# david-cortes/recometrics

Hardware: AMD Instinct MI355X
Metric: users/sec evaluated (all metrics, K=10) (higher is better)
Workload: dtype f32

## Files before the change

recometrics_amd/csrc/rm_launch.hpp:

```cpp
#pragma once
#include "rm_device.hpp"
#include "rm_list.hpp"

namespace rm {

typedef double f64x2 __attribute__((ext_vector_type(2)));
constexpr int GROUP_USERS64 = 16;

struct SweepArgs {
    int n, K;
    int ngt;
    int ext_topk;
    int spec;
    int n_slots, n_groups, n_ublocks;
    int ublock0;
    int n_splits, tiles_total;
    int tail_ublocks, tail_splits, part_splits;
    int part_extra;
    int jmax;
    int list_in_lds;
    int check_nan;
    int buffered_lists;
    int pend_cap, pend_off;
    int sync_off;
    const float4 *Ap, *Bp;
    const int *slot_user, *slot_chunk;
    const int *train_p, *train_i;
    const unsigned *train_bits; int train_words;
    const int *gj; const long long *grow;
    const float *pos_score;
    const int *pos_item;
    unsigned *hist;
    unsigned *thr_shared;
    u32x2 *glists;
    int lane_cap; int *lane_cnt;
    ListEntry *pl;
    PartialStat<float> *pst;
    float *dump;
    int stream_slot0;
    long long stream_ld;
    float *stream_scores;
    const int *noise_row; int noise_row0; const float *noise_E; long long noise_ld;
};

struct Sweep64Args {
    int n, K;
    int ngt;
    int ext_topk;
    int spec;
    int n_slots, n_groups, n_ublocks;
    int ublock0;
// ... 45 lines not shown
```

recometrics_amd/csrc/rm_lib.hip:

```cpp
#include <hip/hip_runtime.h>

#include <algorithm>
#include <array>
#include <cmath>
#include <cstdio>
#include <cstring>
#include <cstdlib>
#include <type_traits>
#include <atomic>
#include <chrono>
#include <condition_variable>
#include <csignal>
#include <functional>
#include <limits>
#include <map>
#include <memory>
#include <mutex>
#include <string>
#include <thread>
#include <vector>

#include "../../include/recometrics_hip.h"
#include "rm_device.hpp"
#include "rm_prep.hpp"
#include "rm_launch.hpp"
#include "rm_finalize.hpp"
#include "rm_noise.hpp"
#include "rm_scores.hpp"

namespace {

using namespace rm;

thread_local std::string g_err;
struct RmError { int code; std::string msg; };

#define HIP_CHECK(expr)                                                                                   \
    do {                                                                                                  \
        hipError_t e_ = (expr);                                                                           \
        if (e_ != hipSuccess)                                                                             \
            throw RmError{e_ == hipErrorOutOfMemory ? RM_ERR_NOMEM : RM_ERR_HIP,                          \
                          std::string(#expr) + ": " + hipGetErrorString(e_)};                             \
    } while (0)

struct Switches {
    bool no_train_bits, no_spec, no_side, ext_topk, no_test_mask, hbm_lists, nsub2, no_pending, no_pos_beside, no_seed, rank_generic,
         no_fused_auc, no_defer_auc, noise_sequential, one_context, noise_per_batch, host_trace, no_pos_flat;
    long long free_mb, stream_budget_mb, noise_budget_mb, lane_cap_min, lane_min_k, lane_cap_set, sample_seed;
    double batch_users;
    std::string splits;
    static bool on(const char *name) { return getenv(name) != nullptr; }
    static long long num(const char *name) { const char *e = getenv(name); return e ? atoll(e) : -1; }
    void load()
    {
        no_train_bits = on("RM_DEBUG_NO_TRAIN_BITS"); no_spec = on("RM_DEBUG_NO_SPEC"); no_side = on("RM_DEBUG_NO_SIDE");
        ext_topk = on("RM_DEBUG_EXT_TOPK"); no_test_mask = on("RM_DEBUG_NO_TEST_MASK");
        hbm_lists = on("RM_DEBUG_HBM_LISTS"); nsub2 = on("RM_DEBUG_NSUB2"); no_pending = on("RM_DEBUG_NO_PENDING");
        no_pos_beside = on("RM_DEBUG_NO_POS_BESIDE"); no_seed = on("RM_DEBUG_NO_SEED");
        rank_generic = on("RM_DEBUG_RANK_GENERIC"); no_fused_auc = on("RM_DEBUG_NO_FUSED_AUC");
        no_defer_auc = on("RM_DEBUG_NO_DEFER_AUC"); noise_sequential = on("RM_DEBUG_NOISE_SEQUENTIAL");
        one_context = on("RM_DEBUG_ONE_CONTEXT"); noise_per_batch = on("RM_DEBUG_NOISE_PER_BATCH"); host_trace = on("RM_HOST_TRACE");
        no_pos_flat = on("RM_DEBUG_NO_POS_FLAT");
        free_mb = num("RM_DEBUG_FREE_MB"); stream_budget_mb = num("RM_STREAM_BUDGET_MB");
        noise_budget_mb = num("RM_NOISE_BUDGET_MB");
        lane_min_k = num("RM_DEBUG_LANE_MIN_K");
        lane_cap_set = num("RM_DEBUG_LANE_CAP");
        sample_seed = num("RM_DEBUG_SAMPLE_SEED");
        lane_cap_min = num("RM_DEBUG_LANE_CAP_MIN");
        const char *b = getenv("RM_BATCH_USERS"); batch_users = b ? atof(b) : 0.0;
        const char *s = getenv("RM_DEBUG_SPLITS"); splits = s ? s : "";
    }
    Switches() { load(); }
};
Switches g_sw;

std::atomic<long long> g_ws_bytes{0};
inline long long debug_free_cap()
{
    return g_sw.free_mb >= 0 ? (g_sw.free_mb << 20) : -1;
}

struct RunTrace {
    std::mutex mu; std::vector<std::pair<const char *, double>> pts; std::chrono::steady_clock::time_point t0 = std::chrono::steady_clock::now();
    void point(const char *what) { std::lock_guard<std::mutex> lk(mu); if (pts.size() > 4096) pts.clear(); pts.emplace_back(what, std::chrono::duration<double, std::milli>(std::chrono::steady_clock::now() - t0).count()); }
};
RunTrace g_run_trace;
#define RM_TRACE_POINT(what) do { if (g_sw.host_trace) g_run_trace.point(what); } while (0)

std::atomic<unsigned long long> g_ws_stamp{1};
struct Workspace {
    struct Buf { void *ptr = nullptr; size_t bytes = 0; unsigned long long stamp = 0; };
    std::map<std::string, Buf> bufs;
    void *get(const std::string &name, size_t bytes)
    {
        bytes = std::max<size_t>(bytes, 256);
// ... 309 lines not shown
{
    return lane_lists_possible<T>(K, three_subtiles) && lane_list_bytes<T>(K, lane_blocks_bound<T>(m)) <= lane_budget_bytes(ws);
}

inline long long dense_row_words(long long n) { return (n + 191) / 192 * 6; }
inline bool dense_rows_fit(const Workspace &ws, int m, long long n)
{
    const long long words = dense_row_words(n);
    if (words > TRAIN_BITS_MAX_WORDS || g_sw.no_train_bits) return false;
    const unsigned long long bytes = (unsigned long long)m * (unsigned long long)words * 4ull;
    if (bytes <= (1ull << 30)) return true;
    if (bytes > (8ull << 30)) return false;
    return (long long)bytes <= free_plus_owned(ws, {"train_bits", "stream_scores", "sel_hi", "sel_lo"}) / 4;
}
template <class C> inline void set_train_bits(SweepArgs &sa, Ctx &cx, const C &c, int m, int n, bool fit, hipStream_t stream, bool mask_test, bool early = false, bool early_masked = false,
                                              unsigned char *ent_masked = nullptr)
{
    Workspace &ws = cx.ws;
    const long long words = dense_row_words(n);
    const size_t bytes = (size_t)m * (size_t)words * 4;
    sa.train_bits = nullptr; sa.train_words = 0;
    if (!fit) { cx.dense.invalidate(); return; }
    unsigned *bits = (unsigned *)ws.get("train_bits", bytes);
    const bool ready = (early && early_masked == mask_test) || (c.same_train_rows && cx.dense.fits(ws, m, words, mask_test));
    if (!ready)
        launch_train_bits(stream, m, n, (int)words, c.train_p, c.train_i, (mask_test || ent_masked) ? c.test_p : nullptr, c.test_i, bits,
                          (const Plan *)ws.get("plan", sizeof(Plan)), c.only_users, ent_masked, mask_test);
    cx.dense.set(ws, words, m, mask_test, ready ? cx.dense.partial : c.only_users != nullptr, c.items_tag, c.train_p);
    sa.train_bits = bits; sa.train_words = (int)words;
}
template <class C> inline void set_train_bits(Sweep64Args &, Ctx &, const C &, int, int, bool, hipStream_t, bool, bool = false, bool = false, unsigned char * = nullptr) {}
inline void set_part_extra(SweepArgs &sa, int extra) { sa.part_extra = extra; }
inline void set_part_extra(Sweep64Args &, int) {}
inline void set_spec(SweepArgs &sa)
{
    sa.spec = (sa.check_nan || sa.noise_E || sa.ext_topk || g_sw.no_spec) ? 0 : (sa.train_bits ? 1 : 2);
}
inline void set_spec(Sweep64Args &sa) { sa.spec = (sa.check_nan || sa.noise_E || sa.ext_topk || g_sw.no_spec) ? 0 : 1; }
inline void set_ext_bits(SweepArgs &sa, const unsigned *bits, int words) { sa.train_bits = bits; sa.train_words = words; }
inline void set_ext_bits(Sweep64Args &, const unsigned *, int) {}

template <class T> inline int sample_seed_items(const Workspace &ws, int K, int n, long long n_slots, bool off, bool lists = false)
{
    if (off || g_sw.sample_seed == 0) return 0;
    int S;
    if (g_sw.sample_seed > 0) {
        S = 64;
        for (int c : {256, 1024, 2048, 4096}) if (g_sw.sample_seed >= c) S = c;
    } else {
        S = K <= 128 ? 1024 : (K <= 384 ? 2048 : 4096);
        if (lists) { if (K < 12) return 0; S = 256; }
        if ((long long)S * 6 > n || K * 2 > S) return 0;
        if (sizeof(T) == 8 && K < 16) return 0;
    }
    if (S > n || K > S) return 0;
    if ((long long)sizeof(T) * n_slots * S > free_plus_owned(ws, {"sample_scores"}) / 8) return 0;
    return S;
}
template <class T, class Args>
inline void seed_from_sample(const Args &sa, Workspace &ws, int S, int NG, int n_slots, int n_ublocks, hipStream_t stream, const void *items64 = nullptr, void *lists = nullptr)
{
    typedef Prec<T> P;
    typedef typename std::remove_pointer<decltype(Args{}.thr_shared)>::type ThrT;
    T *sample = (T *)ws.get("sample_scores", sizeof(T) * (size_t)n_slots * (size_t)S);
    Args sd = sa;
    sd.n = S; sd.tiles_total = S / TILE_ITEMS; sd.K = 1; sd.n_splits = 1; sd.tail_ublocks = 0; sd.tail_splits = 1; sd.part_splits = 1;
// ... 126 lines not shown
        double best = 1e300;
        for (int sct = 1; sct <= max_splits; sct++) {
            const double t1 = last((double)n_ublocks * sct / n_cu) * block(sct);
            if (t1 < best - 1e-9) { best = t1; n_splits = sct; tail_ublocks = 0; tail_splits = 0; }
            const long long full = (long long)n_ublocks * sct / n_cu;
            const int main_ub = (int)(full * n_cu / sct), tail_ub = n_ublocks - main_ub;
            if (full == 0 || tail_ub == 0) continue;
            for (int ts = sct + 1; ts <= max_tail; ts++) {
                const double t2 = (double)main_ub * sct / n_cu * block(sct) + last((double)tail_ub * ts / n_cu) * block(ts);
                if (t2 < best * 0.99) { best = t2; n_splits = sct; tail_ublocks = tail_ub; tail_splits = ts; }
            }
        }
    }
    if (!sw.splits.empty()) {
        int v[3] = {1, 0, 0};
        sscanf(sw.splits.c_str(), "%d,%d,%d", &v[0], &v[1], &v[2]);
        n_splits = std::max(1, std::min(v[0], std::max(1, MAX_PARTS / nsub)));
        tail_ublocks = std::max(0, std::min(v[1], n_ublocks)); tail_splits = std::max(1, std::min(v[2], std::max(1, MAX_PARTS / nsub)));
        if (tail_ublocks == 0) tail_splits = 0;
    }
    g.n_splits = n_splits; g.tail_ublocks = tail_ublocks; g.tail_splits = tail_splits;
    g.part_splits = std::max(n_splits, tail_splits);
    g.mask_test = std::is_same<T, float>::value && want_auc && !ext_topk && !check_nan && hp.n_slots > 0 &&
                  dense_ok && hp.n_slots == hp.n_active && hp.n_only_ndcg == 0 &&
                  nsub * g.part_splits + 1 <= MAX_PARTS && !sw.no_test_mask;
    g.use_ext_bits = c.ext_bits != nullptr && c.ext_words == dense_row_words(n) && (!c.ext_masked || g.mask_test);
    if (g.use_ext_bits) g.mask_test = c.ext_masked;
    g.n_part = nsub * g.part_splits + (g.mask_test ? 1 : 0);
    g.part_extra = g.mask_test ? 1 : 0;
    g.list_in_lds = !ext_topk && !want_lane && lds_need_n(true, nsub) + SYNC_BYTES <= LDS_LIMIT && !sw.hbm_lists;
    g.want_pending = !ext_topk && !want_lane && P::has_pending && !sw.no_pending;
    g.per_key = (size_t)g.n_waves * WAVE * P::pend_key_bytes;
    g.pend_cap = g.want_pending ? P::pend_cap_max : 0;
    g.lds_total = std::min<size_t>(LDS_LIMIT, lds_need_n(g.list_in_lds, nsub) + SYNC_BYTES + g.pend_cap * g.per_key);
    g.sync_off = g.lds_total - SYNC_BYTES;
    g.u_split = 0; g.j_shallow = -1; g.lds_l = 0;
    if (!g.list_in_lds && !want_lane && K <= 32 && want_auc && !sw.hbm_lists) {
        for (int j = g.jmax - 1; j >= 0 && g.j_shallow < 0; j--)
            if (sweep_lds<T>(NG, K, want_auc, true, nsub, j) + SYNC_BYTES <= LDS_LIMIT) g.j_shallow = j;
        if (g.j_shallow >= 0) g.u_split = hp.class_offset[g.j_shallow + 1] / (GROUPS_PER_BLOCK * P::GU);
    }
    if (g.u_split > 0)
        g.lds_l = std::min<size_t>(LDS_LIMIT, sweep_lds<T>(NG, K, want_auc, true, nsub, g.j_shallow) + SYNC_BYTES + g.pend_cap * g.per_key);
    return g;
}

inline Geometry scores_geometry(const Plan &hp, int n, bool want_auc)
{
    Geometry g{};
    g.jmax = want_auc ? hp.jmax : 0;
    g.n_ublocks = (hp.n_groups + GROUPS_PER_BLOCK - 1) / GROUPS_PER_BLOCK;
    g.nsub = 2; g.tile_items = TILE_ITEMS; g.n_waves = 8;
    g.tiles_total = (n + TILE_ITEMS - 1) / TILE_ITEMS;
    g.n_splits = 1; g.part_splits = 1; g.n_part = 1;
    g.u_split = 0; g.j_shallow = -1;
    return g;
}

template <class T>
struct Pipeline {
    typedef Prec<T> P;
    typedef typename std::remove_pointer<decltype(typename P::Args{}.thr_shared)>::type ThrT;
    static constexpr int GU = P::GU;
    const Call<T> &c; hipStream_t stream; Ctx &cx; Workspace &ws;
    const int m, n, k, K;
    const bool use_side = !g_sw.no_side;
    Beside side, pos;
// ... 241 lines not shown
        if (want_auc) positives();

        if (n_stream > 0) stream_scores = (T *)ws.get("stream_scores", sizeof(T) * (size_t)n_stream * (size_t)stream_ld);
        if (!ext_topk) pl = (Entry<T> *)ws.get("pl", sizeof(Entry<T>) * (size_t)n_slots * g.n_part * K);
        pst = (PartialStat<T> *)ws.get("pst", sizeof(PartialStat<T>) * (size_t)n_slots * g.n_part);
        const unsigned n_blocks = (unsigned)((g.n_ublocks - g.tail_ublocks) * g.n_splits + g.tail_ublocks * g.tail_splits);
        lane_lists = want_lane && !ext_topk;
        int lane_cap = lane_lists ? P::lane_cap(K) : 0;
        if (lane_lists && g_sw.lane_cap_set > 0) lane_cap = (int)std::min<long long>(std::max<long long>(P::lane_cap(K), (g_sw.lane_cap_set + 15) / 16 * 16), (COLLECT_MAX_ENTRIES - K) / 16 * 16);
        if (lane_lists && g_sw.lane_cap_min >= 0)
            lane_cap = std::min(lane_cap, (K + lane_sel_slack(K) + 16 + 1 + 15) / 16 * 16);
        if (lane_lists) {
            glists = (typename P::ListT *)ws.get("glists", (size_t)n_blocks * g.n_waves * WAVE * (size_t)lane_cap * (sizeof(T) + 4));
            lane_cnt = (int *)ws.get("lane_cnt", sizeof(int) * (size_t)n_blocks * g.n_waves * WAVE);
        } else if (!g.list_in_lds && !ext_topk) {
            glists = (typename P::ListT *)ws.get("glists", sizeof(typename P::ListT) * (size_t)n_blocks * g.n_waves * GU * (2 * K + 32));
        }

        thr_shared = (ThrT *)ws.get("thr_shared", sizeof(ThrT) * (size_t)n_slots);
        if (want_auc && !ext_topk && !g_sw.no_seed)
            hipLaunchKernelGGL((k_seed_thresholds<T, ThrT>), dim3(cdiv(n_slots, 256)), dim3(256), 0, stream, n_slots, stream_slot0, K, GU, slot_user, slot_chunk,
                               user_nslots, flags, c.test_p, grow, pos_score, spos_score, thr_shared);
        else HIP_CHECK(hipMemsetAsync(thr_shared, 0, sizeof(ThrT) * (size_t)n_slots, stream));
        sa.thr_shared = thr_shared;
        sa.n = n; sa.K = K; sa.ngt = NG; sa.n_slots = n_slots; sa.n_groups = n_groups; sa.n_ublocks = g.n_ublocks;
        sa.n_splits = g.n_splits; sa.tail_ublocks = g.tail_ublocks; sa.tail_splits = g.tail_splits; sa.part_splits = g.part_splits; sa.tiles_total = tiles_total; sa.jmax = g.jmax; sa.check_nan = check_nan ? 1 : 0; sa.buffered_lists = (want_lane || ext_topk) ? 1 : 0; sa.ext_topk = ext_topk ? 1 : 0;
        sa.Ap = (decltype(sa.Ap))Ap; sa.Bp = (decltype(sa.Bp))Bp; sa.slot_user = slot_user; sa.slot_chunk = slot_chunk;
        sa.train_p = c.train_p; sa.train_i = c.train_i; sa.gj = gj; sa.grow = grow;
        sa.pos_score = pos_score; sa.pos_item = pos_item; sa.hist = hist; sa.glists = glists; sa.lane_cap = lane_cap; sa.lane_cnt = lane_cnt; sa.pl = pl; sa.pst = pst; sa.dump = nullptr;
        P::set_pending(sa, g.pend_cap, 0);
        P::set_sync(sa, (int)g.sync_off);
        sa.stream_slot0 = stream_slot0; sa.stream_ld = stream_ld; sa.stream_scores = stream_scores;
        set_part_extra(sa, g.part_extra);
        sa.noise_row = c.noise_row; sa.noise_row0 = c.noise_row0; sa.noise_E = c.noise_E; sa.noise_ld = c.noise_ld;
        set_spec(sa);

        if (side.marked(SIDE_ROWS_AND_PACKS)) side.await(SIDE_ROWS_AND_PACKS, stream);
        const bool sample_lists = !lane_lists && !ext_topk && sizeof(T) == 4;
        const int sample_S = (lane_lists || sample_lists) ? sample_seed_items<T>(ws, K, n, n_slots, check_nan || c.noise_E != nullptr, sample_lists) : 0;
        if (sample_S > 0 && !sample_lists) seed_from_sample<T>(sa, ws, sample_S, NG, n_slots, g.n_ublocks, stream);
        else if (sample_S > 0) {
            const long long units = P::items_units(sample_S / TILE_ITEMS, NG);
            typename P::PackT *Bs = (typename P::PackT *)ws.get("sample_items", 16 * (size_t)units);
            void *Ls = ws.get("sample_lists", sizeof(typename P::ListT) * (size_t)g.n_ublocks * 8 * GU * (2 + 32));
            pack_operands(c.A, c.lda, c.B, c.ldb, sample_S, k, NG, TILE_ITEMS, slot_user, 0, Ap, 0, Bs, units, stream, true);
            seed_from_sample<T>(sa, ws, sample_S, NG, n_slots, g.n_ublocks, stream, Bs, Ls);
        }
        RM_TRACE_POINT("run: preparation enqueued");
    }

    void positives()
    {
        const int n_groups = hp.n_groups;
        const long long rows = hp.total_rows + n_groups;
        pos_score = (T *)ws.get("pos_score", sizeof(T) * (size_t)(rows + 1) * GU);
        pos_item = (int *)ws.get("pos_item", sizeof(int) * (size_t)(rows + 1) * GU);
        hist = (unsigned *)ws.get("hist", sizeof(unsigned) * (size_t)(rows + 1) * GU);
        T *pos_tmp = (T *)ws.get("pos_tmp", sizeof(T) * (size_t)std::max<long long>(c.nnz_test, 1));
        pos_order = (int *)ws.get("pos_order", sizeof(int) * (size_t)std::max<long long>(c.nnz_test, 1));
        PosArgs<T> pa{m, n, k, c.A, c.lda, c.B, c.ldb, c.train_p, c.train_i, c.test_p, c.test_i,
                      flags, user_nslots, uslot_base, slot_index, grow, pos_tmp, pos_order, pos_score, pos_item, GU};
        pa.noise_row = c.noise_row; pa.noise_row0 = c.noise_row0; pa.noise_E = c.noise_E; pa.noise_ld = c.noise_ld;
        pa.noise_flag = c.noise_flag; pa.plan = plan;
        if (sizeof(T) == 4)
            pa.pos_key = (unsigned long long *)ws.get("pos_key", 8 * ((size_t)std::max<long long>(c.nnz_test, 1) + 8));
        const bool flat = flat_early;
// ... 1384 lines not shown
```

recometrics_amd/csrc/rm_sweep.hpp:

```cpp
#pragma once
#include "rm_device.hpp"
#include "rm_list.hpp"
#include "rm_launch.hpp"

namespace rm {

typedef float f32x16 __attribute__((ext_vector_type(16)));

__device__ __forceinline__ float hw_max(float a, float b) { float d; asm("v_max_f32 %0, %1, %2" : "=v"(d) : "v"(a), "v"(b)); return d; }
__device__ __forceinline__ float hw_max3(float a, float b, float c) { float d; asm("v_max3_f32 %0, %1, %2, %3" : "=v"(d) : "v"(a), "v"(b), "v"(c)); return d; }
__device__ __forceinline__ float hw_min3(float a, float b, float c) { float d; asm("v_min3_f32 %0, %1, %2, %3" : "=v"(d) : "v"(a), "v"(b), "v"(c)); return d; }


typedef __attribute__((address_space(3))) unsigned long long *LdsListPtr;
typedef u32x2 *GblListPtr;

typedef __attribute__((address_space(3))) const float *LdsF32Ptr;
typedef __attribute__((address_space(3))) unsigned *LdsU32Ptr;

#define RM_CMP_LT(m, p, x) asm volatile("v_cmp_lt_f32 %0, %1, %2" : "=s"(m) : "v"(p), "v"(x))
#define RM_SEL(d, a, b, m) asm volatile("v_cndmask_b32 %0, %1, %2, %3" : "=v"(d) : "v"(a), "v"(b), "s"(m))
__device__ __forceinline__ float hw_absmin3(float a, float b, float c) { float d; asm("v_min3_f32 %0, |%1|, |%2|, |%3|" : "=v"(d) : "v"(a), "v"(b), "v"(c)); return d; }

template <int J>
__device__ __forceinline__ void auc_pass(const float (&v)[16], unsigned pos_addr,
                                         const int *pos_item_g, int sb, int h, float piv_root, float piv_lo, float piv_hi)
{
    constexpr unsigned HIST_DELTA = (unsigned)GROUPS_PER_BLOCK * (1u << J) * GROUP_USERS * 4u;
    unsigned at[16];
#ifndef RM_TOP_LEVELS
#define RM_TOP_LEVELS 2
#endif
    constexpr int TOP = J >= 2 ? RM_TOP_LEVELS : 0;
    unsigned long long mk0, mk1, mk2;
    if (TOP == 2) {
        constexpr unsigned Q = 128u << (J >= 2 ? J - 2 : 0);
        const unsigned a1 = pos_addr | Q, a2 = pos_addr | (2 * Q), a3 = pos_addr | (3 * Q);
        #pragma unroll
        for (int r = 0; r < 16; r++) at[r] = pos_addr;
        #pragma unroll
        for (int i = 0; i < 48 + 2; i++) {
            if (i < 48) {
                const float pv = i < 16 ? piv_lo : (i < 32 ? piv_root : piv_hi);
                if (i % 3 == 0) RM_CMP_LT(mk0, pv, v[i % 16]); else if (i % 3 == 1) RM_CMP_LT(mk1, pv, v[i % 16]); else RM_CMP_LT(mk2, pv, v[i % 16]);
            }
            if (i >= 2) {
                const int j = i - 2;
                const unsigned tgt = j < 16 ? a1 : (j < 32 ? a2 : a3);
                if (j % 3 == 0) RM_SEL(at[j % 16], at[j % 16], tgt, mk0); else if (j % 3 == 1) RM_SEL(at[j % 16], at[j % 16], tgt, mk1); else RM_SEL(at[j % 16], at[j % 16], tgt, mk2);
            }
        }
    } else if (TOP == 1) {
        const unsigned a2 = pos_addr | (128u << (J >= 1 ? J - 1 : 0));
        #pragma unroll
        for (int i = 0; i < 16 + 2; i++) {
            if (i < 16) { if (i % 3 == 0) RM_CMP_LT(mk0, piv_root, v[i]); else if (i % 3 == 1) RM_CMP_LT(mk1, piv_root, v[i]); else RM_CMP_LT(mk2, piv_root, v[i]); }
            if (i >= 2) {
                const int j = i - 2;
                if (j % 3 == 0) RM_SEL(at[j], pos_addr, a2, mk0); else if (j % 3 == 1) RM_SEL(at[j], pos_addr, a2, mk1); else RM_SEL(at[j], pos_addr, a2, mk2);
            }
        }
    } else {
        #pragma unroll
        for (int r = 0; r < 16; r++) at[r] = pos_addr;
    }
    constexpr int FIRST_ST = J - TOP > 0 ? (1 << (J - TOP - 1)) : 0;
    #pragma unroll
    for (int st = FIRST_ST; st >= 1; st >>= 1) {
        float pv[16];
        #pragma unroll
        for (int r = 0; r < 16; r++) pv[r] = *(LdsF32Ptr)(at[r] + (st - 1) * 128);
        #pragma unroll
        for (int i = 0; i < 16 + 2; i++) {
            if (i == 0) __builtin_amdgcn_s_waitcnt(0xCC7F); else if (i == 4) __builtin_amdgcn_s_waitcnt(0xC87F);
            else if (i == 8) __builtin_amdgcn_s_waitcnt(0xC47F); else if (i == 12) __builtin_amdgcn_s_waitcnt(0xC07F);
            if (i < 16) { if (i % 3 == 0) RM_CMP_LT(mk0, pv[i], v[i]); else if (i % 3 == 1) RM_CMP_LT(mk1, pv[i], v[i]); else RM_CMP_LT(mk2, pv[i], v[i]); }
            if (i >= 2) {
                const int j = i - 2;
                const unsigned cand = at[j] | (unsigned)(st * 128);
                if (j % 3 == 0) RM_SEL(at[j], at[j], cand, mk0); else if (j % 3 == 1) RM_SEL(at[j], at[j], cand, mk1); else RM_SEL(at[j], at[j], cand, mk2);
            }
        }
    }
    float nx[16];
    #pragma unroll
    for (int r = 0; r < 16; r++) nx[r] = *(LdsF32Ptr)(at[r]);
    float df[16];
    #pragma unroll
    for (int r = 0; r < 16; r++) {
        if (r == 0) __builtin_amdgcn_s_waitcnt(0xCC7F); else if (r == 4) __builtin_amdgcn_s_waitcnt(0xC87F);
        else if (r == 8) __builtin_amdgcn_s_waitcnt(0xC47F); else if (r == 12) __builtin_amdgcn_s_waitcnt(0xC07F);
        df[r] = nx[r] - v[r];
    }
    const float m0 = hw_absmin3(df[0], df[1], df[2]), m1 = hw_absmin3(df[3], df[4], df[5]), m2 = hw_absmin3(df[6], df[7], df[8]);
    const float m3 = hw_absmin3(df[9], df[10], df[11]), m4 = hw_absmin3(df[12], df[13], df[14]);
    const float dmin = hw_absmin3(hw_absmin3(m0, m1, m2), hw_absmin3(m3, m4, df[15]), df[15]);
    if (wave_any(dmin == 0.f)) {
        int sb_walk = sb;
        asm volatile("" : "+s"(sb_walk));
        auto walk = [&](int r) {
            if (df[r] == 0.f) {
                const int item = sb_walk + mfma32_row(r, h);
                unsigned t = at[r] - pos_addr;
                while (*(const int *)((const char *)pos_item_g + t) > item) {
                    t += 128;
                    if (!(t < (unsigned)(((1 << J) - 1) * 128) && *(LdsF32Ptr)(pos_addr + t) == v[r])) break;
                }
                at[r] = pos_addr + t;
            }
        };
        if (wave_any(m0 == 0.f)) { walk(0); walk(1); walk(2); }
        if (wave_any(m1 == 0.f)) { walk(3); walk(4); walk(5); }
        if (wave_any(m2 == 0.f)) { walk(6); walk(7); walk(8); }
        if (wave_any(m3 == 0.f)) { walk(9); walk(10); walk(11); }
        if (wave_any(m4 == 0.f)) { walk(12); walk(13); walk(14); }
        if (wave_any(df[15] == 0.f)) walk(15);
    }
    const unsigned one = 1u;
    #pragma unroll
    for (int r = 0; r < 16; r++)
        asm volatile("ds_add_u32 %0, %1 offset:%2" :: "v"(at[r]), "v"(one), "n"(HIST_DELTA) : "memory");
}


template <int NGT, bool AUC, bool DUMP, int LMODE, int NSUB, int SPEC = 0>
__global__ __launch_bounds__(256 * NSUB)
void k_sweep(SweepArgs a)
{
    constexpr int TILE = 32 * NSUB;
    static_assert(SPEC >= 0 && SPEC <= 2 && !(SPEC && DUMP), "unknown specialisation");
    const bool f_bits = SPEC == 1 ? true : (SPEC == 2 ? false : a.train_bits != nullptr);
    const bool f_nan = SPEC ? false : a.check_nan != 0, f_noise = SPEC ? false : a.noise_E != nullptr, f_ext = SPEC ? false : a.ext_topk != 0;
    constexpr int NWAVES = 4 * NSUB, THREADS = 64 * NWAVES;
    constexpr bool LLDS = LMODE == LM_LDS;
    constexpr bool buffered = LMODE == LM_HBM_APPEND;
    constexpr bool NGT_RT = NGT == 0;
    constexpr int NG = NGT_RT ? 16 : (NGT < 16 ? NGT : 16);
    constexpr int NC_CT = NGT_RT ? 0 : NGT / NG;
    const int NGTV = NGT_RT ? a.ngt : NGT;
    const int NC = NGT_RT ? a.ngt / NG : NC_CT;
    constexpr bool AF_RESIDENT = NC_CT == 1;
    constexpr bool AF_PREFETCH = !AF_RESIDENT && LMODE != LM_HBM_APPEND;
    extern __shared__ __attribute__((aligned(16))) char smem[];
    constexpr int BUF_F4 = NG * 2 * TILE;
    const int tid = threadIdx.x, lane = tid & 63, wave = __builtin_amdgcn_readfirstlane(tid >> 6);
    const int gi = wave & 3, sub = wave >> 2;
    const int ul = lane & 31, h = lane >> 5;
    int blk_u, split, nsplit;
    {
        const int n_ub1 = a.n_ublocks - a.tail_ublocks, b1 = n_ub1 * a.n_splits;
        if ((int)blockIdx.x < b1) { blk_u = a.ublock0 + a.n_ublocks - 1 - (int)(blockIdx.x % n_ub1); split = blockIdx.x / n_ub1; nsplit = a.n_splits; }
        else { const int j = (int)blockIdx.x - b1; blk_u = a.ublock0 + a.tail_ublocks - 1 - j % a.tail_ublocks; split = j / a.tail_ublocks; nsplit = a.tail_splits; }
    }
    const int group = blk_u * GROUPS_PER_BLOCK + gi;
    const bool group_ok = group < a.n_groups;
    const int slot = group * GROUP_USERS + ul;
    const bool slot_ok = group_ok && slot < a.n_slots;
    const int K = a.K, n = a.n;

    const int glast = min(a.n_groups, (blk_u + 1) * GROUPS_PER_BLOCK) - 1;
    const int jb = AUC ? a.gj[glast] : 0;
    const int PLb = (1 << jb) - 1;

    float4 *ldsB = (float4 *)smem;
    char *p = smem + 2 * BUF_F4 * 16;
    ListEntry *lists_lds = (ListEntry *)p;
    if (LLDS) p += GROUPS_PER_BLOCK * (K + 2) * GROUP_USERS * (int)sizeof(ListEntry);
    const int PLmax = PLb;
    const unsigned tbytes = (unsigned)(PLmax + 1) * GROUP_USERS * 4;
    p = smem + (((unsigned)(p - smem) + tbytes - 1) / tbytes) * tbytes;
    float *posL = (float *)p;  p += GROUPS_PER_BLOCK * tbytes;
    unsigned *histL = (unsigned *)p;  p += AUC ? GROUPS_PER_BLOCK * tbytes : 0;
    const int pend_room = (a.sync_off - (int)(p - smem)) / (NWAVES * WAVE * 8);
    char *pend_lds = p;

    const int user = slot_ok ? a.slot_user[slot] : -1;
    const bool primary = slot_ok && a.slot_chunk[slot] == 0;
    float thr = primary ? neg_inf_f() : nan_sentinel_f();
    float vmax = neg_inf_f(), vmin = pos_inf_f();
    bool track_min = true;
    unsigned long long nanmask = 0;
    int ntc = 0, nte = 0, nt = IDX_EMPTY, nt2 = IDX_EMPTY;

    const int tiles_per = (a.tiles_total + nsplit - 1) / nsplit;
    const int t0 = split * tiles_per, t1 = min(a.tiles_total, t0 + tiles_per);
    const int ntiles = max(0, t1 - t0);

    const unsigned *tb_row = (a.train_bits && user >= 0) ? a.train_bits + (size_t)user * a.train_words : nullptr;
    unsigned tb_idx = (a.train_bits && user >= 0) ? (unsigned)user * (unsigned)a.train_words + (unsigned)(t0 * NSUB + sub) : 0u;
    if (user >= 0 && !f_bits) {
        ntc = a.train_p[user]; nte = a.train_p[user + 1];
        const int first_item = t0 * TILE;
        int lo = ntc, hi = nte;
        while (lo < hi) { const int mid = (lo + hi) >> 1; if (a.train_i[mid] < first_item) lo = mid + 1; else hi = mid; }
        ntc = lo;
        nt = ntc < nte ? a.train_i[ntc] : IDX_EMPTY;
        nt2 = ntc + 1 < nte ? a.train_i[ntc + 1] : IDX_EMPTY;
    }

    float4 af[NG];
    const float4 *af_src = a.Ap + ((size_t)(group_ok ? group : 0) * NGTV * 2 + h) * GROUP_USERS + ul;
    #pragma unroll
// ... 30 lines not shown
    auto list_release = [&]() {
        if (!LLDS) return;
        if (h == 0) { Lwk[0] = wkey; Lwp[0] = (unsigned long long)wpos; }
        if (lane == 0) __hip_atomic_store(list_lock, 0u, __ATOMIC_RELEASE, __HIP_MEMORY_SCOPE_WORKGROUP);
    };
    const int pend_want = pend_room < a.pend_cap ? pend_room : a.pend_cap;
    const int pend_cap = (buffered || pend_want < 2) ? 0 : pend_want;
    int pcnt = 0;
    LdsListPtr Pp = (LdsListPtr)((unsigned long long *)pend_lds + wave * pend_cap * WAVE + lane);
    auto offer_key = [&](unsigned long long key) {
        if (LLDS) { keylist_offer<GROUP_USERS>(Ll, K, key, wkey, wpos); return; }
        float s; int item;
        unpack_key(key, s, item);
        if (s >= ws) list_offer<float, GROUP_USERS>(Lr, K, s, item, ws, widx, wpos);
    };
    bool merged = false;
    auto merge_pending = [&]() {
        merged = true;
        const int pc = __shfl_xor(pcnt, 32);
        const int lim = h == 0 ? (pcnt > pc ? pcnt : pc) : 0;
        list_acquire();
        for (int i = 0; wave_any(i < lim); i++) {
            if (h == 0) {
                if (i < pcnt) offer_key(Pp[i * WAVE]);
                if (i < pc) offer_key(Pp[i * WAVE + 32]);
            }
        }
        list_release();
        pcnt = 0;
        if (LLDS) ws = (wkey >> 32) ? ord_unkey((unsigned)(wkey >> 32)) : neg_inf_f();
    };

    if (AUC) {
        for (int i = tid; i < GROUPS_PER_BLOCK * (PLb + 1) * GROUP_USERS; i += THREADS) {
            const int g4 = i / ((PLb + 1) * GROUP_USERS), rem = i % ((PLb + 1) * GROUP_USERS);
            const int gg = blk_u * GROUPS_PER_BLOCK + g4;
            posL[g4 * (PLmax + 1) * GROUP_USERS + rem] = gg < a.n_groups ? a.pos_score[(a.grow[gg] + gg) * GROUP_USERS + rem] : pos_inf_f();
        }
        for (int i = tid; i < GROUPS_PER_BLOCK * (PLmax + 1) * GROUP_USERS; i += THREADS) histL[i] = 0;
    }
    const unsigned pos_addr = (unsigned)(size_t)(__attribute__((address_space(3))) const float *)(posL + gi * (PLmax + 1) * GROUP_USERS + ul);
    float piv_root = pos_inf_f(), piv_lo = pos_inf_f(), piv_hi = pos_inf_f();
    if (AUC && jb >= 2) {
        __syncthreads();
        const int r0 = (1 << (jb - 1)) - 1, d = 1 << (jb - 2);
        piv_root = *(LdsF32Ptr)(pos_addr + r0 * 128);
        piv_lo = *(LdsF32Ptr)(pos_addr + (r0 - d) * 128);
        piv_hi = *(LdsF32Ptr)(pos_addr + (r0 + d) * 128);
    }
    const int *pos_item_g = (AUC && group_ok) ? a.pos_item + (a.grow[group] + group) * GROUP_USERS + ul : nullptr;
    const bool stream_lane = slot_ok && slot >= a.stream_slot0;
    const bool wave_streams = wave_any(stream_lane);
    float *stream_row = stream_lane ? a.stream_scores + (size_t)(slot - a.stream_slot0) * (size_t)a.stream_ld : nullptr;
    const float *noise_lane = (a.noise_E && user >= 0)
        ? a.noise_E + (size_t)(a.noise_row ? a.noise_row[user] - a.noise_row0 : user) * (size_t)a.noise_ld : nullptr;

    const unsigned lds_base = (unsigned)(__UINTPTR_TYPE__)(__attribute__((address_space(3))) char *)smem;
    constexpr int STAGE_PIECES = (NG + 3) / 4;
    unsigned stage_voff[STAGE_PIECES];
    #pragma unroll
    for (int j = 0; j < STAGE_PIECES; j++) stage_voff[j] = (unsigned)(((gi + 4 * j) * 2 * TILE + h * TILE + sub * 32 + ul) * 16);
    auto stage = [&](int unit, int buf) {
        const char *src = (const char *)a.Bp + (size_t)unit * (BUF_F4 * 16);
        #pragma unroll
        for (int j = 0; j < STAGE_PIECES; j++) {
            const int g = gi + 4 * j;
            if (NG % 4 == 0 || g < NG) {
                const unsigned m0v = lds_base + (unsigned)((buf * BUF_F4 + (sub * NG + g) * 64) * 16);
                asm volatile("s_mov_b32 m0, %0\n\ts_nop 0\n\tglobal_load_lds_dwordx4 %1, %2"
                             :: "s"(m0v), "v"(stage_voff[j]), "s"(src) : "memory", "m0");
            }
        }
    };

#ifndef RM_FULL_BARRIER
    constexpr bool EARLY_ARRIVE = AF_RESIDENT && NG >= 4 && NG % 2 == 0;
#else
    constexpr bool EARLY_ARRIVE = false;
#endif
    static_assert(!EARLY_ARRIVE || NG % 2 == 0, "early arrival needs an even number of factor groups");
    LdsU32Ptr arrive_p = (LdsU32Ptr)(smem + a.sync_off) + sub;
// ... 208 lines not shown
                const unsigned long long hitm = __ballot(v[r] >= thr);
                if (hitm) {
                    const float other = (hitm >> 32) ? __shfl_xor(v[r], 32) : nan_sentinel_f();
                    if (h == 0 && primary) {
                        const int item0 = sb + mfma32_row(r, 0), item1 = sb + mfma32_row(r, 1);
                        if (LLDS) { if (v[r] >= ws) keylist_offer<GROUP_USERS>(Ll, K, pack_key(v[r], item0), wkey, wpos);
                                    if (other >= ws) keylist_offer<GROUP_USERS>(Ll, K, pack_key(other, item1), wkey, wpos);
                                    ws = (wkey >> 32) ? ord_unkey((unsigned)(wkey >> 32)) : neg_inf_f(); }
                        else      { if (v[r] >= ws) list_offer<float, GROUP_USERS>(Lr, K, v[r], item0, ws, widx, wpos);
                                    if (other >= ws) list_offer<float, GROUP_USERS>(Lr, K, other, item1, ws, widx, wpos); }
                    }
                }
            }
            list_release();
        }
        if (!buffered && cm && (!pend_cap || merged)) {
            merged = false;
            const float t2 = __shfl(ws, ul);
            if (primary) {
                thr = t2 > thr ? t2 : thr;
                const unsigned kk = ord_key(t2);
                if (h == 0 && kk > thr_pub) { atomicMax(a.thr_shared + slot, kk); }
                thr_pub = kk > thr_pub ? kk : thr_pub;
            }
        }
        if (wave_streams) {
            if (stream_lane) {
                #pragma unroll
                for (int q4 = 0; q4 < 4; q4++)
                    *(float4 *)(stream_row + sb + 8 * q4 + 4 * h) = make_float4(v[4 * q4], v[4 * q4 + 1], v[4 * q4 + 2], v[4 * q4 + 3]);
            }
        }
        if (AUC) {
            switch (jb) {
                case 1: auc_pass<1>(v, pos_addr, pos_item_g, sb, h, piv_root, piv_lo, piv_hi); break;
                case 2: auc_pass<2>(v, pos_addr, pos_item_g, sb, h, piv_root, piv_lo, piv_hi); break;
                case 3: auc_pass<3>(v, pos_addr, pos_item_g, sb, h, piv_root, piv_lo, piv_hi); break;
                case 4: auc_pass<4>(v, pos_addr, pos_item_g, sb, h, piv_root, piv_lo, piv_hi); break;
                case 5: auc_pass<5>(v, pos_addr, pos_item_g, sb, h, piv_root, piv_lo, piv_hi); break;
                case 6: auc_pass<6>(v, pos_addr, pos_item_g, sb, h, piv_root, piv_lo, piv_hi); break;
                default: break;
            }
        }
        if (buffered) {
            const bool own = wave_any(lb_off >= lb_trig_now);
            unsigned ep = __builtin_amdgcn_readfirstlane(*sel_epoch);
            if (own || (ep != sel_seen && wave_any(lb_off >= lb_half))) {
                if (own && ep == sel_seen) {
                    if (lane == 0) asm volatile("ds_add_u32 %0, %1" :: "v"((unsigned)(__UINTPTR_TYPE__)sel_epoch), "v"(1u) : "memory");
                    ep++;
                }
                lane_bounds();
                lb_trig_now = lb_trigger;
            }
            sel_seen = ep;
        }
    };

    f32x16 acc;
    const int nunits = ntiles * NC;
    constexpr unsigned SYNC_WAVES = 4;
    LdsU32Ptr arrive = (LdsU32Ptr)(smem + a.sync_off) + sub;
    if (tid < (buffered ? 8 : 4)) ((LdsU32Ptr)(smem + a.sync_off))[tid] = 0u;
    if (ntiles > 0) stage(t0 * NC, 0);
    unsigned tile_bits = (tb_row && ntiles > 0) ? a.train_bits[tb_idx] >> (4 * h) : 0u;
    __builtin_amdgcn_s_waitcnt(WAIT_VMCNT0);
    __syncthreads();
    auto load_thr = [&]() -> unsigned {
        return (primary && !DUMP) ? __hip_atomic_load(a.thr_shared + slot, __ATOMIC_RELAXED, __HIP_MEMORY_SCOPE_AGENT) : 0u;
    };
    unsigned thr_seen = load_thr();
    for (int i = 0; i < ntiles; i++) {
        unsigned thr_next = thr_seen;
// ... 16 lines not shown
                const int sub_s = __builtin_amdgcn_readfirstlane(sub);
                const unsigned mine = sub_s == 0 ? c0 : (sub_s == 1 ? c1 : c2);
                const unsigned o1 = sub_s == 0 ? c1 : c0, o2 = (NSUB == 3) ? (sub_s == 2 ? c1 : c2) : o1;
                const bool behind = mine + 2 < o1 || mine + 2 < o2, ahead = mine > o1 + 2 && mine > o2 + 2;
                if (behind) __builtin_amdgcn_s_setprio(2);
                else if (ahead) __builtin_amdgcn_s_setprio(0);
                else __builtin_amdgcn_s_setprio(1);
            }
#endif
            if (unit + 1 < nunits) stage(t0 * NC + unit + 1, (unit + 1) & 1);
            if (c == 0) thr_next = load_thr();
            unsigned bits_next = 0u;
            if (c == NC - 1 && tb_row && i + 1 < ntiles) { tb_idx += NSUB; bits_next = a.train_bits[tb_idx]; }
            do_mfma(acc, unit & 1, c, tile_bits);
#ifndef RM_FULL_BARRIER
            __builtin_amdgcn_s_waitcnt(WAIT_VMCNT0);
            if (!EARLY_ARRIVE && lane == 0) asm volatile("ds_add_u32 %0, %1" :: "v"((unsigned)(__UINTPTR_TYPE__)arrive), "v"(1u) : "memory");
#endif
            if (c == NC - 1) do_epi(acc, t0 + i, thr_seen, tile_bits);
            if (c == NC - 1) tile_bits = bits_next >> (4 * h);
#if defined(RM_FULL_BARRIER)
            __builtin_amdgcn_s_waitcnt(WAIT_VMCNT0);
            __syncthreads();
#endif
        }
        thr_seen = thr_next;
    }
    if (DUMP) return;
    if (pend_cap) merge_pending();
    if (LLDS) __syncthreads();

    {
    const SweepArgs &a = *late_kernargs<SweepArgs>();
    const int n_part = a.part_splits * NSUB + a.part_extra;
    const int part = split * NSUB + sub;
    {
        const float omax = __shfl_xor(vmax, 32), omin = __shfl_xor(vmin, 32);
        vmax = __builtin_fmaxf(vmax, omax); vmin = __builtin_fminf(vmin, omin);
        const bool hn = ((nanmask >> ul) & 1ull) | ((nanmask >> (ul + 32)) & 1ull);
        if (slot_ok && h == 0) {
            PartialStat<float> ps;
            ps.vmax = vmax; ps.vmin = vmin; ps.rocsum = 0; ps.has_nan = hn ? 1 : 0; ps.pad = 0;
            a.pst[(size_t)slot * n_part + part] = ps;
            ListEntry *dst = a.pl + ((size_t)slot * n_part + part) * K;
            if (LLDS && sub == 0) { keylist_sort_desc<GROUP_USERS>(Ll, K); for (int i = 0; i < K; i++) unpack_key(Ll[i * GROUP_USERS], dst[i].s, dst[i].idx); }
            if (LLDS && sub != 0) { dst[0].s = neg_inf_f(); dst[0].idx = IDX_EMPTY; }
            if (split == 0) for (int sp = nsplit; sp < a.part_splits; sp++) {
                ps.vmax = neg_inf_f(); ps.vmin = pos_inf_f(); ps.has_nan = 0;
                a.pst[(size_t)slot * n_part + sp * NSUB + sub] = ps;
                ListEntry *de = a.pl + ((size_t)slot * n_part + sp * NSUB + sub) * K;
                if (a.pl) { de[0].s = neg_inf_f(); de[0].idx = IDX_EMPTY; }
            }
        }
    }
    if (AUC && a.part_extra && split == 0 && sub == 0 && h == 0 && slot_ok && slot < a.stream_slot0) {
        const int pe = n_part - 1;
        ListEntry *dx = a.pl + ((size_t)slot * n_part + pe) * K;
        const unsigned hcol = (unsigned)(size_t)(__attribute__((address_space(3))) unsigned *)(histL + gi * (PLmax + 1) * GROUP_USERS + ul);
        float bmax = neg_inf_f(), bmin = pos_inf_f();
        int filled = 0;
        for (int i = PLb - 1; i >= 0; i--) {
            const float x = *(LdsF32Ptr)(pos_addr + (unsigned)i * 128u);
            if (x < pos_inf_f()) {
                if (filled == 0) bmax = x;
                bmin = x;
                asm volatile("ds_add_u32 %0, %1" :: "v"(hcol + (unsigned)i * 128u), "v"(1u) : "memory");
                if (filled < K) { dx[filled].s = x; dx[filled].idx = pos_item_g[i * GROUP_USERS]; }
                filled++;
            }
        }
        for (int i = filled; i < K; i++) { dx[i].s = neg_inf_f(); dx[i].idx = IDX_EMPTY; }
        PartialStat<float> ps;
        ps.vmax = bmax; ps.vmin = bmin; ps.rocsum = 0; ps.has_nan = 0; ps.pad = 0;
        a.pst[(size_t)slot * n_part + pe] = ps;
    }
    if (!LLDS && !buffered) {
        if (slot_ok && h == 0) {
            ListEntry *dst = a.pl + ((size_t)slot * n_part + part) * K;
            list_sort_desc<float, GROUP_USERS>(Lr, K);
            for (int i = 0; i < K; i++) ListRaw<float>::unpack(Lr[i * GROUP_USERS], dst[i].s, dst[i].idx);
        }
    } else if (!LLDS && !a.ext_topk) {
        a.lane_cnt[((size_t)blockIdx.x * NWAVES + wave) * WAVE + lane] = (slot_ok && primary) ? (int)(lb_off >> 9) : 0;
    }
    if (AUC) {
        __builtin_amdgcn_s_waitcnt(0xC07F);
        __syncthreads();
        for (int i = tid; i < GROUPS_PER_BLOCK * (PLb + 1) * GROUP_USERS; i += THREADS) {
            const int g4 = i / ((PLb + 1) * GROUP_USERS), rem = i % ((PLb + 1) * GROUP_USERS);
            const int gg = blk_u * GROUPS_PER_BLOCK + g4;
            const unsigned c = histL[g4 * (PLmax + 1) * GROUP_USERS + rem];
            if (gg < a.n_groups && c) atomicAdd(&a.hist[(a.grow[gg] + gg) * GROUP_USERS + rem], c);
        }
    }
    }
}

}
```

Measured before the change: 17.73 million.

## Store AUC positive-score table as score/next-address pairs for branchless binary search

Result: no change. 17.80 million (median of 4 runs) (+0.4%).

```diff
diff --git a/recometrics_amd/csrc/rm_launch.hpp b/recometrics_amd/csrc/rm_launch.hpp
--- a/recometrics_amd/csrc/rm_launch.hpp
+++ b/recometrics_amd/csrc/rm_launch.hpp
@@ -17,6 +17,7 @@
     int n_splits, tiles_total;
     int tail_ublocks, tail_splits, part_splits;
     int part_extra;
+    int rank_plain;
     int jmax;
     int list_in_lds;
     int check_nan;
diff --git a/recometrics_amd/csrc/rm_lib.hip b/recometrics_amd/csrc/rm_lib.hip
--- a/recometrics_amd/csrc/rm_lib.hip
+++ b/recometrics_amd/csrc/rm_lib.hip
@@ -45,7 +45,7 @@
 
 struct Switches {
     bool no_train_bits, no_spec, no_side, ext_topk, no_test_mask, hbm_lists, nsub2, no_pending, no_pos_beside, no_seed, rank_generic,
-         no_fused_auc, no_defer_auc, noise_sequential, one_context, noise_per_batch, host_trace, no_pos_flat;
+         no_fused_auc, no_defer_auc, noise_sequential, one_context, noise_per_batch, host_trace, no_pos_flat, rank_plain;
     long long free_mb, stream_budget_mb, noise_budget_mb, lane_cap_min, lane_min_k, lane_cap_set, sample_seed;
     double batch_users;
     std::string splits;
@@ -61,6 +61,7 @@
         no_defer_auc = on("RM_DEBUG_NO_DEFER_AUC"); noise_sequential = on("RM_DEBUG_NOISE_SEQUENTIAL");
         one_context = on("RM_DEBUG_ONE_CONTEXT"); noise_per_batch = on("RM_DEBUG_NOISE_PER_BATCH"); host_trace = on("RM_HOST_TRACE");
         no_pos_flat = on("RM_DEBUG_NO_POS_FLAT");
+        rank_plain = on("RM_DEBUG_RANK_PLAIN");
         free_mb = num("RM_DEBUG_FREE_MB"); stream_budget_mb = num("RM_STREAM_BUDGET_MB");
         noise_budget_mb = num("RM_NOISE_BUDGET_MB");
         lane_min_k = num("RM_DEBUG_LANE_MIN_K");
@@ -436,6 +437,8 @@
 template <class C> inline void set_train_bits(Sweep64Args &, Ctx &, const C &, int, int, bool, hipStream_t, bool, bool = false, bool = false, unsigned char * = nullptr) {}
 inline void set_part_extra(SweepArgs &sa, int extra) { sa.part_extra = extra; }
 inline void set_part_extra(Sweep64Args &, int) {}
+inline void set_rank_plain(SweepArgs &sa) { sa.rank_plain = g_sw.rank_plain ? 1 : 0; }
+inline void set_rank_plain(Sweep64Args &) {}
 inline void set_spec(SweepArgs &sa)
 {
     sa.spec = (sa.check_nan || sa.noise_E || sa.ext_topk || g_sw.no_spec) ? 0 : (sa.train_bits ? 1 : 2);
@@ -628,7 +631,14 @@
     g.want_pending = !ext_topk && !want_lane && P::has_pending && !sw.no_pending;
     g.per_key = (size_t)g.n_waves * WAVE * P::pend_key_bytes;
     g.pend_cap = g.want_pending ? P::pend_cap_max : 0;
-    g.lds_total = std::min<size_t>(LDS_LIMIT, lds_need_n(g.list_in_lds, nsub) + SYNC_BYTES + g.pend_cap * g.per_key);
+    size_t lds_tables = lds_need_n(g.list_in_lds, nsub);
+    auto with_pairs = [&](size_t plain, int j) {
+        if (!std::is_same<T, float>::value || !want_auc || sw.rank_plain || j < 1 || j > 5) return plain;
+        const size_t up = sweep_lds<T>(NG, K, want_auc, g.list_in_lds, nsub, j + 1);
+        return up + SYNC_BYTES <= LDS_LIMIT ? up : plain;
+    };
+    lds_tables = with_pairs(lds_tables, g.jmax);
+    g.lds_total = std::min<size_t>(LDS_LIMIT, lds_tables + SYNC_BYTES + g.pend_cap * g.per_key);
     g.sync_off = g.lds_total - SYNC_BYTES;
     g.u_split = 0; g.j_shallow = -1; g.lds_l = 0;
     if (!g.list_in_lds && !want_lane && K <= 32 && want_auc && !sw.hbm_lists) {
@@ -936,6 +946,7 @@
         P::set_sync(sa, (int)g.sync_off);
         sa.stream_slot0 = stream_slot0; sa.stream_ld = stream_ld; sa.stream_scores = stream_scores;
         set_part_extra(sa, g.part_extra);
+        set_rank_plain(sa);
         sa.noise_row = c.noise_row; sa.noise_row0 = c.noise_row0; sa.noise_E = c.noise_E; sa.noise_ld = c.noise_ld;
         set_spec(sa);
 
diff --git a/recometrics_amd/csrc/rm_sweep.hpp b/recometrics_amd/csrc/rm_sweep.hpp
--- a/recometrics_amd/csrc/rm_sweep.hpp
+++ b/recometrics_amd/csrc/rm_sweep.hpp
@@ -22,19 +22,26 @@
 #define RM_SEL(d, a, b, m) asm volatile("v_cndmask_b32 %0, %1, %2, %3" : "=v"(d) : "v"(a), "v"(b), "s"(m))
 __device__ __forceinline__ float hw_absmin3(float a, float b, float c) { float d; asm("v_min3_f32 %0, |%1|, |%2|, |%3|" : "=v"(d) : "v"(a), "v"(b), "v"(c)); return d; }
 
-template <int J>
+typedef __attribute__((address_space(3))) const u32x2 *LdsPairPtr;
+
+template <int J, bool PAIR>
 __device__ __forceinline__ void auc_pass(const float (&v)[16], unsigned pos_addr,
                                          const int *pos_item_g, int sb, int h, float piv_root, float piv_lo, float piv_hi)
 {
-    constexpr unsigned HIST_DELTA = (unsigned)GROUPS_PER_BLOCK * (1u << J) * GROUP_USERS * 4u;
+    constexpr unsigned ROW = PAIR ? 256u : 128u;
+    constexpr unsigned HIST_DELTA = (unsigned)GROUPS_PER_BLOCK * (1u << J) * ROW;
+    static_assert(HIST_DELTA <= 65535u, "the histogram's distance is an immediate offset");
     unsigned at[16];
 #ifndef RM_TOP_LEVELS
 #define RM_TOP_LEVELS 2
 #endif
-    constexpr int TOP = J >= 2 ? RM_TOP_LEVELS : 0;
-    unsigned long long mk0, mk1, mk2;
+#ifndef RM_TOP_LEVELS_PAIR
+#define RM_TOP_LEVELS_PAIR 0
+#endif
+    constexpr int TOP = J >= 2 ? (PAIR ? RM_TOP_LEVELS_PAIR : RM_TOP_LEVELS) : 0;
+    unsigned long long mk0, mk1, mk2, mk3;
     if (TOP == 2) {
-        constexpr unsigned Q = 128u << (J >= 2 ? J - 2 : 0);
+        constexpr unsigned Q = ROW << (J >= 2 ? J - 2 : 0);
         const unsigned a1 = pos_addr | Q, a2 = pos_addr | (2 * Q), a3 = pos_addr | (3 * Q);
         #pragma unroll
         for (int r = 0; r < 16; r++) at[r] = pos_addr;
@@ -51,7 +58,7 @@
             }
         }
     } else if (TOP == 1) {
-        const unsigned a2 = pos_addr | (128u << (J >= 1 ? J - 1 : 0));
+        const unsigned a2 = pos_addr | (ROW << (J >= 1 ? J - 1 : 0));
         #pragma unroll
         for (int i = 0; i < 16 + 2; i++) {
             if (i < 16) { if (i % 3 == 0) RM_CMP_LT(mk0, piv_root, v[i]); else if (i % 3 == 1) RM_CMP_LT(mk1, piv_root, v[i]); else RM_CMP_LT(mk2, piv_root, v[i]); }
@@ -65,6 +72,35 @@
         for (int r = 0; r < 16; r++) at[r] = pos_addr;
     }
     constexpr int FIRST_ST = J - TOP > 0 ? (1 << (J - TOP - 1)) : 0;
+    if (PAIR) {
+        #pragma unroll
+        for (int st = FIRST_ST; st >= 1; st >>= 1) {
+            #pragma unroll
+            for (int hf = 0; hf < 2; hf++) {
+                u32x2 pr[8];
+                #pragma unroll
+                for (int r = 0; r < 8; r++) pr[r] = *(LdsPairPtr)(at[8 * hf + r] + (st - 1) * 256);
+#ifndef RM_PAIR_MASKS
+#define RM_PAIR_MASKS 4
+#endif
+                constexpr int LAG = RM_PAIR_MASKS - 1;
+                #pragma unroll
+                for (int i = 0; i < 8 + LAG; i++) {
+                    if (i == 0) __builtin_amdgcn_s_waitcnt(0xC47F); else if (i == 4) __builtin_amdgcn_s_waitcnt(0xC07F);
+                    if (i < 8) {
+                        const float pv = __uint_as_float(pr[i].x), x = v[8 * hf + i];
+                        const int m = i % RM_PAIR_MASKS;
+                        if (m == 0) RM_CMP_LT(mk0, pv, x); else if (m == 1) RM_CMP_LT(mk1, pv, x); else if (m == 2) RM_CMP_LT(mk2, pv, x); else RM_CMP_LT(mk3, pv, x);
+                    }
+                    if (i >= LAG) {
+                        const int j = i - LAG, q = 8 * hf + j, m = j % RM_PAIR_MASKS;
+                        if (m == 0) RM_SEL(at[q], at[q], pr[j].y, mk0); else if (m == 1) RM_SEL(at[q], at[q], pr[j].y, mk1);
+                        else if (m == 2) RM_SEL(at[q], at[q], pr[j].y, mk2); else RM_SEL(at[q], at[q], pr[j].y, mk3);
+                    }
+                }
+            }
+        }
+    } else {
     #pragma unroll
     for (int st = FIRST_ST; st >= 1; st >>= 1) {
         float pv[16];
@@ -81,6 +117,7 @@
                 if (j % 3 == 0) RM_SEL(at[j], at[j], cand, mk0); else if (j % 3 == 1) RM_SEL(at[j], at[j], cand, mk1); else RM_SEL(at[j], at[j], cand, mk2);
             }
         }
+    }
     }
     float nx[16];
     #pragma unroll
@@ -102,9 +139,9 @@
             if (df[r] == 0.f) {
                 const int item = sb_walk + mfma32_row(r, h);
                 unsigned t = at[r] - pos_addr;
-                while (*(const int *)((const char *)pos_item_g + t) > item) {
-                    t += 128;
-                    if (!(t < (unsigned)(((1 << J) - 1) * 128) && *(LdsF32Ptr)(pos_addr + t) == v[r])) break;
+                while (*(const int *)((const char *)pos_item_g + (PAIR ? t >> 1 : t)) > item) {
+                    t += ROW;
+                    if (!(t < (unsigned)((1 << J) - 1) * ROW && *(LdsF32Ptr)(pos_addr + t) == v[r])) break;
                 }
                 at[r] = pos_addr + t;
             }
@@ -166,8 +203,17 @@
     char *p = smem + 2 * BUF_F4 * 16;
     ListEntry *lists_lds = (ListEntry *)p;
     if (LLDS) p += GROUPS_PER_BLOCK * (K + 2) * GROUP_USERS * (int)sizeof(ListEntry);
-    const int PLmax = PLb;
-    const unsigned tbytes = (unsigned)(PLmax + 1) * GROUP_USERS * 4;
+    unsigned tbytes = (unsigned)(PLb + 1) * GROUP_USERS * 4;
+    bool pairs = false;
+    if (AUC && !a.rank_plain && jb >= 1 && jb <= 5) {
+        const unsigned tb2 = 2 * tbytes;
+        const int end2 = (int)((((unsigned)(p - smem) + tb2 - 1) / tb2) * tb2 + 2 * GROUPS_PER_BLOCK * tb2);
+        const int room2 = (a.sync_off - end2) / (NWAVES * WAVE * 8);
+        pairs = end2 <= a.sync_off && (buffered || room2 >= (a.pend_cap < 3 ? a.pend_cap : 3));
+        if (pairs) tbytes = tb2;
+    }
+    const unsigned row_b = pairs ? 256u : 128u;
+    const int jsel = pairs ? jb + 8 : jb;
     p = smem + (((unsigned)(p - smem) + tbytes - 1) / tbytes) * tbytes;
     float *posL = (float *)p;  p += GROUPS_PER_BLOCK * tbytes;
     unsigned *histL = (unsigned *)p;  p += AUC ? GROUPS_PER_BLOCK * tbytes : 0;
@@ -264,21 +310,27 @@
     };
 
     if (AUC) {
+        const unsigned pos_base = (unsigned)(size_t)(__attribute__((address_space(3))) const float *)posL;
         for (int i = tid; i < GROUPS_PER_BLOCK * (PLb + 1) * GROUP_USERS; i += THREADS) {
             const int g4 = i / ((PLb + 1) * GROUP_USERS), rem = i % ((PLb + 1) * GROUP_USERS);
             const int gg = blk_u * GROUPS_PER_BLOCK + g4;
-            posL[g4 * (PLmax + 1) * GROUP_USERS + rem] = gg < a.n_groups ? a.pos_score[(a.grow[gg] + gg) * GROUP_USERS + rem] : pos_inf_f();
-        }
-        for (int i = tid; i < GROUPS_PER_BLOCK * (PLmax + 1) * GROUP_USERS; i += THREADS) histL[i] = 0;
-    }
-    const unsigned pos_addr = (unsigned)(size_t)(__attribute__((address_space(3))) const float *)(posL + gi * (PLmax + 1) * GROUP_USERS + ul);
+            const float x = gg < a.n_groups ? a.pos_score[(a.grow[gg] + gg) * GROUP_USERS + rem] : pos_inf_f();
+            if (pairs) {
+                u32x2 e;
+                e.x = __float_as_uint(x); e.y = pos_base + (unsigned)i * 8u + 256u;
+                ((u32x2 *)posL)[i] = e;
+            } else posL[i] = x;
+        }
+        for (int i = tid; i < (int)(GROUPS_PER_BLOCK * tbytes / 4); i += THREADS) histL[i] = 0;
+    }
+    const unsigned pos_addr = (unsigned)(size_t)(__attribute__((address_space(3))) const float *)posL + (unsigned)gi * tbytes + (unsigned)ul * (pairs ? 8u : 4u);
     float piv_root = pos_inf_f(), piv_lo = pos_inf_f(), piv_hi = pos_inf_f();
     if (AUC && jb >= 2) {
         __syncthreads();
         const int r0 = (1 << (jb - 1)) - 1, d = 1 << (jb - 2);
-        piv_root = *(LdsF32Ptr)(pos_addr + r0 * 128);
-        piv_lo = *(LdsF32Ptr)(pos_addr + (r0 - d) * 128);
-        piv_hi = *(LdsF32Ptr)(pos_addr + (r0 + d) * 128);
+        piv_root = *(LdsF32Ptr)(pos_addr + r0 * row_b);
+        piv_lo = *(LdsF32Ptr)(pos_addr + (r0 - d) * row_b);
+        piv_hi = *(LdsF32Ptr)(pos_addr + (r0 + d) * row_b);
     }
     const int *pos_item_g = (AUC && group_ok) ? a.pos_item + (a.grow[group] + group) * GROUP_USERS + ul : nullptr;
     const bool stream_lane = slot_ok && slot >= a.stream_slot0;
@@ -553,13 +605,18 @@
             }
         }
         if (AUC) {
-            switch (jb) {
-                case 1: auc_pass<1>(v, pos_addr, pos_item_g, sb, h, piv_root, piv_lo, piv_hi); break;
-                case 2: auc_pass<2>(v, pos_addr, pos_item_g, sb, h, piv_root, piv_lo, piv_hi); break;
-                case 3: auc_pass<3>(v, pos_addr, pos_item_g, sb, h, piv_root, piv_lo, piv_hi); break;
-                case 4: auc_pass<4>(v, pos_addr, pos_item_g, sb, h, piv_root, piv_lo, piv_hi); break;
-                case 5: auc_pass<5>(v, pos_addr, pos_item_g, sb, h, piv_root, piv_lo, piv_hi); break;
-                case 6: auc_pass<6>(v, pos_addr, pos_item_g, sb, h, piv_root, piv_lo, piv_hi); break;
+            switch (jsel) {
+                case 1: auc_pass<1, false>(v, pos_addr, pos_item_g, sb, h, piv_root, piv_lo, piv_hi); break;
+                case 2: auc_pass<2, false>(v, pos_addr, pos_item_g, sb, h, piv_root, piv_lo, piv_hi); break;
+                case 3: auc_pass<3, false>(v, pos_addr, pos_item_g, sb, h, piv_root, piv_lo, piv_hi); break;
+                case 4: auc_pass<4, false>(v, pos_addr, pos_item_g, sb, h, piv_root, piv_lo, piv_hi); break;
+                case 5: auc_pass<5, false>(v, pos_addr, pos_item_g, sb, h, piv_root, piv_lo, piv_hi); break;
+                case 6: auc_pass<6, false>(v, pos_addr, pos_item_g, sb, h, piv_root, piv_lo, piv_hi); break;
+                case 9: auc_pass<1, true>(v, pos_addr, pos_item_g, sb, h, piv_root, piv_lo, piv_hi); break;
+                case 10: auc_pass<2, true>(v, pos_addr, pos_item_g, sb, h, piv_root, piv_lo, piv_hi); break;
+                case 11: auc_pass<3, true>(v, pos_addr, pos_item_g, sb, h, piv_root, piv_lo, piv_hi); break;
+                case 12: auc_pass<4, true>(v, pos_addr, pos_item_g, sb, h, piv_root, piv_lo, piv_hi); break;
+                case 13: auc_pass<5, true>(v, pos_addr, pos_item_g, sb, h, piv_root, piv_lo, piv_hi); break;
                 default: break;
             }
         }
@@ -642,6 +699,8 @@
 
     {
     const SweepArgs &a = *late_kernargs<SweepArgs>();
+    const bool pairs = jsel >= 8;
+    const unsigned row_b = pairs ? 256u : 128u, tbytes = row_b << jb;
     const int n_part = a.part_splits * NSUB + a.part_extra;
     const int part = split * NSUB + sub;
     {
@@ -666,15 +725,15 @@
     if (AUC && a.part_extra && split == 0 && sub == 0 && h == 0 && slot_ok && slot < a.stream_slot0) {
         const int pe = n_part - 1;
         ListEntry *dx = a.pl + ((size_t)slot * n_part + pe) * K;
-        const unsigned hcol = (unsigned)(size_t)(__attribute__((address_space(3))) unsigned *)(histL + gi * (PLmax + 1) * GROUP_USERS + ul);
+        const unsigned hcol = pos_addr + (unsigned)GROUPS_PER_BLOCK * tbytes;
         float bmax = neg_inf_f(), bmin = pos_inf_f();
         int filled = 0;
         for (int i = PLb - 1; i >= 0; i--) {
-            const float x = *(LdsF32Ptr)(pos_addr + (unsigned)i * 128u);
+            const float x = *(LdsF32Ptr)(pos_addr + (unsigned)i * row_b);
             if (x < pos_inf_f()) {
                 if (filled == 0) bmax = x;
                 bmin = x;
-                asm volatile("ds_add_u32 %0, %1" :: "v"(hcol + (unsigned)i * 128u), "v"(1u) : "memory");
+                asm volatile("ds_add_u32 %0, %1" :: "v"(hcol + (unsigned)i * row_b), "v"(1u) : "memory");
                 if (filled < K) { dx[filled].s = x; dx[filled].idx = pos_item_g[i * GROUP_USERS]; }
                 filled++;
             }
@@ -699,7 +758,7 @@
         for (int i = tid; i < GROUPS_PER_BLOCK * (PLb + 1) * GROUP_USERS; i += THREADS) {
             const int g4 = i / ((PLb + 1) * GROUP_USERS), rem = i % ((PLb + 1) * GROUP_USERS);
             const int gg = blk_u * GROUPS_PER_BLOCK + g4;
-            const unsigned c = histL[g4 * (PLmax + 1) * GROUP_USERS + rem];
+            const unsigned c = histL[pairs ? 2 * i : i];
             if (gg < a.n_groups && c) atomicAdd(&a.hist[(a.grow[gg] + gg) * GROUP_USERS + rem], c);
         }
     }
```
